# tingiskhan/pyfilter

Measured on AMD Instinct MI355X. Metric: particle-steps/sec (batch x particles x T), 1M-particle APF, higher is better.
Workload: dtype f32; 1 GPU; apf_lgo_1m: APF + lgo proposal, systematic resampling, N=1048576 particles x B=1 filters per GPU, T=250, state dim 1; parallelism=single GPU

## Files before the change

### pyfilter_amd/csrc/pf_fused.hpp

```cpp
#pragma once

namespace pf {

#define PF_STEP_B blockIdx.x
#define PF_STEP_K blockIdx.y

#ifdef PF_DEVTOOLS
#define PF_CUT(a, n) ((a).debug_cut == (n))
#define PF_STAMP(a, slot)                                                                       \
    do {                                                                                        \
        if ((a).debug_cut < 0 && !(a).finalize_only && PF_STEP_K == (unsigned)(-(a).debug_cut - 1) &&  \
            PF_STEP_B == 0 && threadIdx.x == 0)                                                 \
            (a).dbg[slot] = (unsigned long long)clock64();                                      \
    } while (0)
#else
#define PF_CUT(a, n) false
#ifdef PF_ISA_MARKS
#define PF_STAMP(a, slot) asm volatile("; PF_MARK " #slot)
#else
#define PF_STAMP(a, slot) do { } while (0)
#endif
#endif

template <typename T> struct FusedArgs {
// ... 383 lines not shown
    for (int r = 0; r < g.rounds_per_tile; ++r) {
        const int64_t r0 = base + (int64_t)r * g.round_elems;
        if (r0 >= g.N) break;
        ++rk;
        const int64_t i0 = r0 + threadIdx.x * VEC;
        const bool on = i0 < g.N;
        T rw[VEC];
#pragma unroll
        for (int j = 0; j < VEC; ++j) rw[j] = -Lim<T>::inf();
        if (on) {
            T lw[VEC], xv[D][VEC];
            if (VEC == 1) lw[0] = lw_col[i0]; else load_vec<T, VEC>(lw_col + i0, lw);
#pragma unroll
            for (int d = 0; d < D; ++d) {
                const T* xc = x_base + ((int64_t)d * g.B + b) * g.N + i0;
                if (VEC == 1) xv[d][0] = xc[0]; else load_vec<T, VEC>(xc, xv[d]);
            }
            T pre[VEC];
#pragma unroll
            for (int j = 0; j < VEC; ++j) {
                T xj[D];
#pragma unroll
                for (int d = 0; d < D; ++d) xj[d] = xv[d][j];
                UserMS<T, D> um = UserMS<T, D>::none();
                if (user && pre_on) {
                    um.gather(a.user_loc, a.user_scale, (int64_t)b * g.N, (int64_t)g.B * g.N, i0 + j, a.user_scale_percol != 0, b, g.B);
                    um.euler(xj, a.user_dt);
                }
                pre[j] = pre_on ? pre_weight<T, D>(a.md, a.proposal, cp, cc, xj, false, um) : T(0);
                if (pre_on && is_nan_or_posinf(pre[j])) acc.poison = true;
                rw[j] = pre_on ? sanitize_logw(pre[j] + lw[j]) : lw[j];
            }
            T e_unused[VEC];
            acc.template push_round<VEC>(lw, xv, false, pre, piv, e_unused);
            if (a.resampler == PF_RESAMPLE_MULTINOMIAL) {
                T ev[VEC];
                draw_exponentials<T, VEC>(a.seed + (a.seed_dev ? *a.seed_dev : 0ull), PF_STREAM_MULTINOMIAL, (uint32_t)a.step,
                                          (uint64_t)((int64_t)b * g.N + i0), ev);
#pragma unroll
                for (int j = 0; j < VEC; ++j) acc.es += (double)ev[j];
            }
        }
        chunk_scan_round<T, VEC>(rw, on, l_col + r0, threadIdx.x * VEC, r * PF_NWAVES + (threadIdx.x >> 6), use_lds ? crec : nullptr, ct_tile);
    }
    T M1, M2, F1, F2;
    acc.template finish<true>(a.part_w(a.step), b, k, g.B, g.tiles, false, red, redm, &a.poison[(a.step & 3) * g.B + b], M1, M2, F1, F2, [](T, T) {}, []() {});
    double Mc, Sc;
    finalize_chunk_table<T>(ct_tile, use_lds ? crec : nullptr, rk * PF_NWAVES, reds, redm, Mc, Sc);
    if (threadIdx.x == 0) {
        const int64_t stride = (int64_t)g.B * g.tiles, o = (int64_t)b * g.tiles + k;
        if (pre_on) {
            a.part_w(a.step)[PQ_M2 * stride + o] = Mc;
            a.part_w(a.step)[PQ_S2 * stride + o] = Sc;
        } else {
            a.part_w(a.step)[PQ_S1 * stride + o] = Sc;
        }
    }
    if (g.rounds_per_tile == 1) {
        __syncthreads();
        const int64_t i0 = base + threadIdx.x * VEC;
        if (i0 < g.N) {
            const double* cg = ct_tile + 2 * (threadIdx.x >> 6);
            const double C = cg[0], gq = cg[1];
            T v[VEC];
            if (VEC == 1) v[0] = l_col[i0]; else load_vec<T, VEC>(l_col + i0, v);
#pragma unroll
            for (int j = 0; j < VEC; ++j) v[j] = (T)(C + gq * (double)v[j]);
            if (VEC == 1) l_col[i0] = v[0]; else store_vec<T, VEC>(l_col + i0, v);
        }
    }
}

#define PF_COMBINE_ITERS (PF_MAX_TILES / PF_BLOCK)
template <typename T> __device__ __forceinline__ double pf_rcp_tot(double tot) {
    if constexpr (sizeof(T) == 4) {
        double r = __builtin_amdgcn_rcp(tot);
        r = __builtin_fma(__builtin_fma(-tot, r, 1.0), r, r);
        r = __builtin_fma(__builtin_fma(-tot, r, 1.0), r, r);
        return r;
    }
    return 1.0 / tot;
}
#define PF_PROBE_STEP 8
struct ColSums {
    double M, S, Q;
};
template <bool WITH_Q, int NX> struct ColPartials {
    double m[PF_COMBINE_ITERS], s[PF_COMBINE_ITERS], q[PF_COMBINE_ITERS];
    double x[NX ? NX : 1][PF_COMBINE_ITERS];
};
template <bool WITH_Q, int NX = 0>
__device__ __forceinline__ void load_col_partials(const double* part, int64_t stride, int64_t cb, int tiles, int slot_m,
                                                  int slot_s, int slot_x, ColPartials<WITH_Q, NX>& r) {
    const int IT = (tiles + PF_BLOCK - 1) / PF_BLOCK;
    if constexpr (PF_COMBINE_ITERS == 4 && NX == 0) {
        if (IT == 4 && (tiles & 3) == 0) {
            const int t0 = threadIdx.x * 4;
            if (t0 < tiles) {
                double a2[2], b2[2];
                const double* pm = part + slot_m * stride + cb + t0;
                load_vec<double, 2>(pm, a2); load_vec<double, 2>(pm + 2, b2);
                r.m[0] = a2[0]; r.m[1] = a2[1]; r.m[2] = b2[0]; r.m[3] = b2[1];
                const double* ps = part + slot_s * stride + cb + t0;
                load_vec<double, 2>(ps, a2); load_vec<double, 2>(ps + 2, b2);
                r.s[0] = a2[0]; r.s[1] = a2[1]; r.s[2] = b2[0]; r.s[3] = b2[1];
                if constexpr (WITH_Q) {
                    const double* pq = part + PQ_Q1 * stride + cb + t0;
                    load_vec<double, 2>(pq, a2); load_vec<double, 2>(pq + 2, b2);
                    r.q[0] = a2[0]; r.q[1] = a2[1]; r.q[2] = b2[0]; r.q[3] = b2[1];
                } else {
                    r.q[0] = r.q[1] = r.q[2] = r.q[3] = 0.0;
                }
            } else {
#pragma unroll
                for (int q = 0; q < 4; ++q) { r.m[q] = -__builtin_huge_val(); r.s[q] = 0.0; r.q[q] = 0.0; }
            }
            return;
        }
    }
#pragma unroll
    for (int q = 0; q < PF_COMBINE_ITERS; ++q) {
        const int t = threadIdx.x * IT + q;
        const bool on = q < IT && t < tiles;
        r.m[q] = on ? part[slot_m * stride + cb + t] : -__builtin_huge_val();
        r.s[q] = on ? part[slot_s * stride + cb + t] : 0.0;
        r.q[q] = (WITH_Q && on) ? part[PQ_Q1 * stride + cb + t] : 0.0;
#pragma unroll
        for (int i = 0; i < NX; ++i) r.x[i][q] = on ? part[(slot_x + i) * stride + cb + t] : 0.0;
    }
}
template <typename T, bool WITH_Q, bool TABLE, int NX = 0>
__device__ __forceinline__ ColSums column_sums(const ColPartials<WITH_Q, NX>& in, int tiles, double* ptl, double* ftl,
                                               double* redm, double* reds, double* X = nullptr) {
#pragma clang fp contract(off)
    const int lane = threadIdx.x & 63, wid = threadIdx.x >> 6;
    const int IT = (tiles + PF_BLOCK - 1) / PF_BLOCK;
    const double (&mloc)[PF_COMBINE_ITERS] = in.m;
    const double (&sloc)[PF_COMBINE_ITERS] = in.s;
    const double (&qloc)[PF_COMBINE_ITERS] = in.q;
    const double (&xloc)[NX ? NX : 1][PF_COMBINE_ITERS] = in.x;
    T mymax_t = -Lim<T>::inf();
#pragma unroll
    for (int q = 0; q < PF_COMBINE_ITERS; ++q) mymax_t = (T)mloc[q] > mymax_t ? (T)mloc[q] : mymax_t;
    const double MR = (double)block_max<T>(mymax_t, reinterpret_cast<T*>(redm));
    double incl[PF_COMBINE_ITERS], ef[PF_COMBINE_ITERS], run = 0.0, qs = 0.0;
    double xs[NX ? NX : 1];
#pragma unroll
    for (int i = 0; i < NX; ++i) xs[i] = 0.0;
#pragma unroll
    for (int q = 0; q < PF_COMBINE_ITERS; ++q) {
        ef[q] = exp_diff_t<T>(mloc[q], MR);
        run += sloc[q] * ef[q];
        incl[q] = run;
        if (WITH_Q) qs += qloc[q] * ef[q] * ef[q];
#pragma unroll
        for (int i = 0; i < NX; ++i) xs[i] += xloc[i][q] * ef[q];
    }
    const double incl_w = wave_scan_incl(run, lane);
    const double qw = WITH_Q ? wave_sum(qs) : 0.0;
#pragma unroll
    for (int i = 0; i < NX; ++i) xs[i] = wave_sum(xs[i]);
    __syncthreads();
    if (lane == 63) reds[wid] = incl_w;
    if (WITH_Q && lane == 0) reds[PF_NWAVES + wid] = qw;
    if (NX && lane == 0) {
#pragma unroll
// ... 123 lines not shown
    }
    double mv[2 * D];
    ColPartials<true, 2 * D> p1;
    ColPartials<false, 0> p2;
    load_col_partials<true, 2 * D>(a.part_r(), stride, cb, g.tiles, PQ_M1, PQ_S1, PQ_MX, p1);
    if (two) load_col_partials<false, 0>(a.part_r(), stride, cb, g.tiles, PQ_M2, PQ_S2, 0, p2);
    const ColSums c1 = column_sums<T, true, false, 2 * D>(p1, g.tiles, nullptr, nullptr, redm, red, mv);
    ColSums c2{0.0, 1.0, 0.0};
    if (two) c2 = column_sums<T, false, false>(p2, g.tiles, nullptr, nullptr, redm, red);
    const double lse_w = c1.M + log(c1.S);
    const double ess = c1.S * c1.S / c1.Q;
    bool resample = apf ? obs : (ess < a.thr_abs);
    if (a.finalize_only) resample = false;
    if (threadIdx.x == 0) {
#pragma unroll
        for (int d = 0; d < D; ++d) {
            const double dm = mv[d] / c1.S;
            double var = mv[D + d] / c1.S - dm * dm;
            if (var < 0.0) var = 0.0;
            a.means[((int64_t)step * g.B + b) * D + d] = (T)(piv[d] + dm);
            a.vars[((int64_t)step * g.B + b) * D + d] = (T)var;
        }
        if (step > 0 && !st.ll_done) {
            double ll = 0.0;
            if (st.prev_observed) {
                ll = lse_w - st.base_lse;
                if (poisoned) ll = __builtin_nan("");
            }
            a.poison[pslot * g.B + b] = 0;
            a.ll_steps[(int64_t)(step - 1) * g.B + b] = (T)ll;
            a.ll_total[b] = (T)(ll_tot + ll);
        }
        st.lse_w = lse_w;
        if (!a.finalize_only) st.resample = resample ? 1 : 0;
        st.ll_done = a.finalize_only ? 1 : 0;
        if (!a.finalize_only) {
            st.prev_observed = obs ? 1 : 0;
            st.base_lse = apf ? a.logN - ((c2.M + log(c2.S)) - lse_w) : (resample ? a.logN : lse_w);
        }
        a.stat[b] = st;
    }
}

template <typename T, int D>
__global__ __launch_bounds__(PF_BLOCK) void k_fused_book(FusedArgs<T> a) {
    __shared__ double red[(2 + 2 * D) * PF_NWAVES];
    __shared__ double redm[PF_NWAVES];
    column_bookkeeping<T, D>(a, blockIdx.y, red, redm);
}

#define PF_WAVES_D1_GENERIC 4
#define PF_WAVES_D1_MN 3
#define PF_WAVES_DN_A 3
template <typename T, int D, int MODE, int PROP, bool FAST, int SPEC, bool MULTI> struct StepWaves {
    static constexpr int value = sizeof(T) != 4 ? 1
                                 : (D == 1 && MODE == 1 && MULTI) ? PF_WAVES_D1_MN
                                 : D == 1     ? (FAST ? 4 : PF_WAVES_D1_GENERIC)
                                 : PROP == PF_PROP_LGO ? 2
                                 : (MODE == 1 || SPEC == 2) ? PF_WAVES_DN_A
                                 : 3;
};
template <typename T, int D, int VEC> struct StepShared {
    static constexpr int WIN = SearchWin<T, VEC>::WIN;
    static constexpr bool XWIN = (sizeof(T) * D <= 8);
    T* win;
    T* xwin;
    int* sh_j0;
    int* sh_cl;
    int* sh_wm;
    double* red;
    double* reds;
    T* redm;
    double* ptl;
    double* ftl;
    int* sh_plan;
    double* crec;
};
template <typename T> struct StepPlan {
    int j0, kt0;
    T ub;
    double offE, invE;
    bool resample;
    bool have_z0;
};
template <typename T, int D, int VEC, int MODE, int SPEC, bool EARLY_Z, bool MULTI>
__device__ __forceinline__ StepPlan<T> step_prologue(const FusedArgs<T>& a, const StepShared<T, D, VEC>& sh, T (&z0)[VEC][D]) {
    const Geom& g = a.g;
    const int b = PF_STEP_B, k = a.tile_of_row(PF_STEP_K);
    const int step = a.step;
    const bool obs = SPEC ? true : a.is_obs();
    const bool apf = SPEC ? (SPEC == 1) : (a.filter == PF_FILTER_APF);
    const bool two = apf && obs;
    StepPlan<T> pl{0, 0, T(0), 0.0, 0.0, false, false};
    PF_STAMP(a, 0);
#ifdef PF_DEVTOOLS
    if (a.debug_cut < 0 && threadIdx.x == 0 && b == 0 && (k % 128) == 0 && k / 128 < 8) a.dbg[16 + k / 128] = wall_clock64();
#endif
    if (apf && !obs) return pl;
    constexpr bool multinomial = MODE == 1;
    const uint64_t seed = a.seed + (a.seed_dev ? *a.seed_dev : 0ull);
    const T u_taped = (!multinomial && a.u_tape) ? a.u_tape[(int64_t)step * g.B + b] : T(0);
    const int64_t stride = (int64_t)g.B * g.tiles;
    const int64_t cb = (int64_t)b * g.tiles;
    double* const redm_d = sh.red + 2 * PF_NWAVES;
    T e0[1] = {T(0)};
    if constexpr (multinomial) {
        T tail[1];
        draw_exponentials<T, 1>(seed, PF_STREAM_MULTINOMIAL, (uint32_t)step, (uint64_t)((int64_t)g.B * g.N + b), tail);
        spacing_table(a.part_r(), stride, cb, g.tiles, (double)tail[0], sh.ptl, sh.reds);
        pl.offE = sh.ptl[k];
        pl.invE = 1.0 / sh.ptl[g.tiles + 1];
        draw_exponentials<T, 1>(seed, PF_STREAM_MULTINOMIAL, (uint32_t)step, (uint64_t)((int64_t)b * g.N + (int64_t)k * g.tile_elems), e0);
    }
    ColPartials<true, 0> p1;
    ColPartials<false, 0> p2;
    constexpr bool SHORT = MULTI;
    const bool one_tile = SHORT && g.tiles == 1 && a.debug_cut != 77;
    double m1 = 0.0, s1 = 0.0, q1 = 0.0;
    if (one_tile) {
        const double* part = a.part_r();
        m1 = part[(two ? PQ_M2 : PQ_M1) * stride + cb];
        s1 = part[(two ? PQ_S2 : PQ_S1) * stride + cb];
        q1 = two ? 0.0 : part[PQ_Q1 * stride + cb];
    }
    const bool few_tiles = SHORT && !one_tile && g.tiles <= PF_WAVE && a.debug_cut != 79;
    if (!one_tile && !few_tiles) {
        if (two) load_col_partials<false, 0>(a.part_r(), stride, cb, g.tiles, PQ_M2, PQ_S2, 0, p2);
        else load_col_partials<true, 0>(a.part_r(), stride, cb, g.tiles, PQ_M1, PQ_S1, 0, p1);
    }
    if (EARLY_Z && (SPEC || !a.z_tape)) {
        const int64_t i0 = (int64_t)k * g.tile_elems + threadIdx.x * VEC;
        if (i0 < g.N) draw_normals<T, D, VEC>(seed, PF_STREAM_NORMAL, (uint32_t)step, (uint64_t)((int64_t)b * g.N + i0), z0);
        pl.have_z0 = true;
    }
    if (one_tile) {
        if (two) {
            column_sums_one_tile<T, false>(m1, s1, q1, sh.ptl, sh.ftl);
            pl.resample = true;
        } else {
            const ColSums c = column_sums_one_tile<T, true>(m1, s1, q1, sh.ptl, sh.ftl);
            pl.resample = c.S * c.S / c.Q < a.thr_abs;
        }
    } else if (few_tiles) {
        if (two) {
            column_sums_wave<T, false>(a.part_r(), stride, cb, g.tiles, PQ_M2, PQ_S2, sh.ptl, sh.ftl);
            pl.resample = true;
        } else {
            const ColSums c = column_sums_wave<T, true>(a.part_r(), stride, cb, g.tiles, PQ_M1, PQ_S1, sh.ptl, sh.ftl);
            pl.resample = c.S * c.S / c.Q < a.thr_abs;
        }
    } else if (two) {
        column_sums<T, false, true>(p2, g.tiles, sh.ptl, sh.ftl, redm_d, sh.red);
        pl.resample = true;
    } else {
        const ColSums c = column_sums<T, true, true>(p1, g.tiles, sh.ptl, sh.ftl, redm_d, sh.red);
        pl.resample = c.S * c.S / c.Q < a.thr_abs;
    }
    PF_STAMP(a, 1);
    if (!pl.resample) return pl;
    const double* ptl = sh.ptl;
    T p;
    if constexpr (multinomial) {
        p = (T)((pl.offE + (double)e0[0]) * pl.invE);
    } else {
        pl.ub = a.u_tape ? u_taped : uniform_draw<T>(seed, PF_STREAM_UNIFORM, (uint32_t)step, (uint64_t)b);
        p = grid_position<T>((int64_t)k * g.tile_elems, pl.ub, T(g.N));
    }
    if (one_tile && a.debug_cut != 78) {
        pl.j0 = 0;
        pl.kt0 = 0;
        return pl;
    }
    if (threadIdx.x < PF_WAVE) {
        const int lane = threadIdx.x;
        int lo = 0, hi = g.tiles - 1;
        while (lo < hi) {
            const int len = hi - lo + 1;
            const int st = (len + PF_WAVE - 1) / PF_WAVE;
            int probe = lo + (lane + 1) * st - 1;
            if (probe > hi) probe = hi;
            const bool ge = (probe >= g.tiles - 1) || !((T)ptl[probe + 1] < p);
            const unsigned long long bal = __ballot(ge);
            const int f = bal ? __ffsll((long long)bal) - 1 : PF_WAVE - 1;
            int nhi = lo + (f + 1) * st - 1;
            if (nhi > hi) nhi = hi;
            lo = lo + f * st;
            if (lo > nhi) lo = nhi;
            hi = nhi;
        }
        const int kt = lo;
        const double Pk = ptl[kt], Pn = ptl[kt + 1], fk = sh.ftl[kt];
        const int64_t first = (int64_t)kt * g.tile_elems;
        const int64_t last = (first + g.tile_elems < g.N ? first + g.tile_elems : g.N) - 1;
        const T* l_col = ((step & 1) ? a.pos : a.cdf) + (int64_t)b * g.N;
        const int64_t len = last + 1 - first;
        auto cdf_at = [&](int64_t q) -> T {
            if constexpr (MULTI) {
                const double* cg = a.ctab_r(b) + 2 * (q / (PF_WAVE * VEC));
                return cdf_from_local<T>(l_col[q], cg[0], cg[1], Pk, fk, Pn, q == last, q == g.N - 1);
            } else {
                return cdf_from_local<T>(l_col[q], Pk, fk, Pn, q == last, q == g.N - 1);
            }
        };
        int64_t res;
        bool found;
        {
            float fr = (float)((double)p - Pk) * __builtin_amdgcn_rcpf((float)(Pn - Pk));
            fr = __builtin_fminf(__builtin_fmaxf(fr, 0.0f), 1.0f);
            int64_t g0 = first + (int64_t)(fr * (float)len) - (PF_WAVE / 2) * PF_PROBE_STEP;
            const int64_t g0max = last - (PF_WAVE - 1) * PF_PROBE_STEP;
            if (g0 > g0max) g0 = g0max;
            if (g0 < first) g0 = first;
            int64_t q = g0 + (int64_t)lane * PF_PROBE_STEP;
            if (q > last) q = last;
            const unsigned long long bal = __ballot(cdf_at(q) >= p);
            const int f = bal ? __ffsll((long long)bal) - 1 : 0;
            found = bal != 0 && (f > 0 || g0 == first);
            res = f > 0 ? g0 + (int64_t)(f - 1) * PF_PROBE_STEP + 1 : first;
        }
        if (!found) {
            const int64_t st = (len + PF_WAVE - 1) / PF_WAVE;
            int64_t probe = first + (lane + 1) * st - 1;
            if (probe > last) probe = last;
            const unsigned long long bal = __ballot(cdf_at(probe) >= p);
            const int f = bal ? __ffsll((long long)bal) - 1 : PF_WAVE - 1;
            res = first + (int64_t)f * st;
            if (res > last) res = last;
        }
        if (lane == 0) {
            sh.sh_plan[0] = (int)res;
            sh.sh_plan[1] = kt;
        }
    }
    __syncthreads();
    pl.j0 = sh.sh_plan[0];
    pl.kt0 = sh.sh_plan[1];
    PF_STAMP(a, 2);
    return pl;
}
template <typename T, int D, int VEC, int MODE, int PROP, bool FAST, int SPEC, int MK, bool RS, bool MULTI>
__device__ __forceinline__ void step_body(const FusedArgs<T>& a, const StepShared<T, D, VEC>& sh, const StepPlan<T>& pl,
                                          const T (&z0)[VEC][D]) {
    const int proposal = (PROP >= 0) ? PROP : a.proposal;
    ModelDesc md = a.md;
    if constexpr (!FAST && MK == 1) { md.hid_kind = PF_HID_VERHULST_EM; md.obs_kind = PF_OBS_SV; md.obs_dim = 1; }
    if constexpr (!FAST && MK == 4) { md.hid_kind = PF_HID_LORENZ63_EM; md.obs_kind = PF_OBS_LINEAR; }
    constexpr bool USER = !FAST && MK == 3;
    constexpr int WIN = StepShared<T, D, VEC>::WIN;
    constexpr int V1 = (MODE == 0) ? 1 : VEC;
    constexpr int STAGED = PF_BLOCK * (VEC + V1);
    constexpr bool XWIN = StepShared<T, D, VEC>::XWIN;
    T* const win = sh.win;
    T* const xwin = sh.xwin;
    int& sh_j0 = *sh.sh_j0;
// ... 23 lines not shown
    const double offE = pl.offE, invE = pl.invE;
    double carryE = 0.0;
    const uint64_t seed = a.seed + (a.seed_dev ? *a.seed_dev : 0ull);
    const T* z_step = (!SPEC && a.z_tape) ? a.z_tape + (int64_t)step * D * g.B * g.N : nullptr;

    ColParams<T, D> cp;
    ColConsts<T, D> cc;
    FastCol<T> fc;
    if constexpr (!FAST && D > 1) {
        load_col_params<T, D>(a, b, step, obs, cp);
        if (pre_next) cp.load_next(a.y + ((int64_t)(step + 1) * a.y_rows + (a.y_rows == 1 ? 0 : b)) * a.md.obs_dim);
    }
    const T ub = pl.ub;

    const T* x_in = a.x[slot];
    const T* lw_in = a.logw[slot] + (int64_t)b * g.N;
#ifdef PF_DEVTOOLS
    T* lw_out = a.logw[slot ^ 1] + (int64_t)b * g.N;
    int32_t* anc_col = a.anc + (int64_t)b * g.N;
#endif
    const T* cdf_col = ((step & 1) ? a.pos : a.cdf) + (int64_t)b * g.N;
    const int64_t base = (int64_t)k * g.tile_elems;
    const T nT = T(N);
    const T rcN = a.rcN;
    const bool pow2 = (N & (N - 1)) == 0;

    bool poison = false;
    PartialAcc<T, D, SPEC != 1> acc;
    acc.init();
    PF_STAMP(a, 9);
    const double* ptab_col = sh.ptl;
    const double* ftab_col = sh.ftl;
    CdfView<T> view;
    view.L = cdf_col;
    view.ptab = ptab_col;
    view.ftab = ftab_col;
    const double* const ct_col = MULTI ? a.ctab_r(b) : nullptr;
    view.ct = ct_col;
    view.chunk_elems = PF_WAVE * VEC;
    view.N = N;
    view.tile_elems = g.tile_elems;
    view.tiles = g.tiles;

    T e_rw[VEC];
    T rwn[VEC];
#pragma unroll
    for (int j = 0; j < VEC; ++j) {
        e_rw[j] = T(0);
        rwn[j] = -Lim<T>::inf();
    }
    const bool scan_next = !apf || pre_next;
    constexpr bool single = !MULTI;
    const bool use_lds = g.rounds_per_tile * PF_NWAVES <= PF_LDS_CHUNKS;
    double* const ct_tile = a.ctab_w(step + 1, b) + 2 * (int64_t)k * g.rounds_per_tile * PF_NWAVES;
    T* const l_next = ((step & 1) ? a.cdf : a.pos) + (int64_t)b * g.N;
    int rk = 0;
    for (int r = 0; r < g.rounds_per_tile; ++r) {
        const int64_t r0 = base + (int64_t)r * g.round_elems;
        if (r0 >= g.N) break;
        const int64_t i0 = r0 + tid * VEC;
        const bool on = i0 < g.N;
        if (MODE == 0 && windowed) {
            int zero[VEC];
#pragma unroll
            for (int j = 0; j < VEC; ++j) zero[j] = 0;
            if (VEC == 1) hd[tid] = 0; else store_vec<int, VEC>(hd + tid * VEC, zero);
        }
        T pv[VEC];
        if (multinomial && windowed) {
            T ev[VEC];
            double incl[VEC], local = 0.0, total;
            if (on) draw_exponentials<T, VEC>(seed, PF_STREAM_MULTINOMIAL, (uint32_t)step, (uint64_t)((int64_t)b * g.N + i0), ev);
#pragma unroll
            for (int j = 0; j < VEC; ++j) {
                local += on ? (double)ev[j] : 0.0;
                incl[j] = local;
            }
            const double excl = block_scan_excl(local, reds, total);
#pragma unroll
            for (int j = 0; j < VEC; ++j) pv[j] = (T)((offE + carryE + excl + incl[j]) * invE);
            carryE += total;
        }

        const int ws = j0 - (j0 % VEC);
        T c0[VEC], c1[V1], xa[D][VEC], xb[D][V1];
        const int ja = ws + tid * VEC, jb = ws + PF_BLOCK * VEC + tid * V1;
        const bool ina = windowed && ja < N, inb = windowed && jb < N;
        if (ina) {
            if (VEC == 1) c0[0] = cdf_col[ja]; else load_vec<T, VEC>(cdf_col + ja, c0);
            if (XWIN) {
#pragma unroll
                for (int d = 0; d < D; ++d) {
                    const T* xc = x_in + ((int64_t)d * g.B + b) * g.N + ja;
                    if (VEC == 1) xa[d][0] = xc[0]; else load_vec<T, VEC>(xc, xa[d]);
                }
            }
        }
        if (inb) {
            if (V1 == 1) c1[0] = cdf_col[jb]; else load_vec<T, V1>(cdf_col + jb, c1);
            if (XWIN) {
#pragma unroll
                for (int d = 0; d < D; ++d) {
                    const T* xc = x_in + ((int64_t)d * g.B + b) * g.N + jb;
                    if (V1 == 1) xb[d][0] = xc[0]; else load_vec<T, V1>(xc, xb[d]);
                }
            }
        }
        T lw_old[VEC];
        if (on && !resample) {
            if (VEC == 1) lw_old[0] = lw_in[i0]; else load_vec<T, VEC>(lw_in + i0, lw_old);
        }

        T zt[VEC][D];
        if (on) {
            if (z_step) {
#pragma unroll
                for (int d = 0; d < D; ++d) {
                    T zr[VEC];
                    const T* zc = z_step + ((int64_t)d * g.B + b) * g.N + i0;
                    if (VEC == 1) zr[0] = zc[0]; else load_vec<T, VEC>(zc, zr);
#pragma unroll
                    for (int j = 0; j < VEC; ++j) zt[j][d] = zr[j];
                }
            } else if (r == 0 && pl.have_z0) {
#pragma unroll
                for (int j = 0; j < VEC; ++j)
#pragma unroll
                    for (int d = 0; d < D; ++d) zt[j][d] = z0[j][d];
            } else {
                draw_normals<T, D, VEC>(seed, PF_STREAM_NORMAL, (uint32_t)step, (uint64_t)((int64_t)b * g.N + i0), zt);
            }
        }
        PF_STAMP(a, 10);
#ifdef PF_DEVTOOLS
        if (PF_CUT(a, 4)) {
            if (on) lw_out[i0] = zt[0][0] + zt[VEC - 1][D - 1];
            continue;
        }
#endif

        int idx[VEC];
        if (windowed) {
            auto map_window = [&](int w0, int wja, int wjb, bool wina, bool winb, T (&m0)[VEC], T (&m1)[V1]) {
                const int te = g.tile_elems;
                while ((unsigned)((kt0 + 1) * te) <= (unsigned)w0) ++kt0;
                int kta = kt0, ktb = kt0;
                {
                    const unsigned e1 = (unsigned)(kt0 + 1) * te, e2 = e1 + te, e3 = e2 + te;
                    kta += ((unsigned)wja >= e1) + ((unsigned)wja >= e2) + ((unsigned)wja >= e3);
                    ktb += ((unsigned)wjb >= e1) + ((unsigned)wjb >= e2) + ((unsigned)wjb >= e3);
                    if (!wina) kta = kt0;
                    if (!winb) ktb = kt0;
                }
                const double tPa = ptab_col[kta], tNa = ptab_col[kta + 1], tFa = ftab_col[kta];
                const double tPb = ptab_col[ktb], tNb = ptab_col[ktb + 1], tFb = ftab_col[ktb];
                const unsigned ea = (unsigned)(kta + 1) * te, eb = (unsigned)(ktb + 1) * te;
                const int la = (int)(ea < (unsigned)N ? ea : (unsigned)N) - 1;
                const int lb = (int)(eb < (unsigned)N ? eb : (unsigned)N) - 1;
                if constexpr (MULTI) {
                    const double* cga = ct_col + 2 * ((wina ? wja : 0) / (PF_WAVE * VEC));
                    const double* cgb = ct_col + 2 * ((winb ? wjb : 0) / (PF_WAVE * VEC));
                    const double Ca = cga[0], ga = cga[1], Cb = cgb[0], gb = cgb[1];
#pragma unroll
                    for (int j = 0; j < VEC; ++j) {
                        const bool tl = (j == VEC - 1) && (wja + j == la);
                        m0[j] = wina ? cdf_from_local<T>(m0[j], Ca, ga, tPa, tFa, tNa, tl, tl && (wja + j == N - 1)) : Lim<T>::inf();
                    }
#pragma unroll
                    for (int j = 0; j < V1; ++j)
                        m1[j] = winb ? cdf_from_local<T>(m1[j], Cb, gb, tPb, tFb, tNb, wjb + j == lb, wjb + j == N - 1) : Lim<T>::inf();
                } else {
#pragma unroll
                    for (int j = 0; j < VEC; ++j) {
                        const bool tl = (j == VEC - 1) && (wja + j == la);
                        m0[j] = wina ? cdf_from_local<T>(m0[j], tPa, tFa, tNa, tl, tl && (wja + j == N - 1)) : Lim<T>::inf();
                    }
#pragma unroll
                    for (int j = 0; j < V1; ++j)
                        m1[j] = winb ? cdf_from_local<T>(m1[j], tPb, tFb, tNb, wjb + j == lb, wjb + j == N - 1) : Lim<T>::inf();
                }
            };
            map_window(ws, ja, jb, ina, inb, c0, c1);
            if (XWIN) {
#pragma unroll
                for (int d = 0; d < D; ++d) {
                    if (ina) { if (VEC == 1) xwin[d * WIN + tid] = xa[d][0]; else store_vec<T, VEC>(xwin + d * WIN + tid * VEC, xa[d]); }
                    if (inb) { if (V1 == 1) xwin[d * WIN + PF_BLOCK * VEC + tid] = xb[d][0]; else store_vec<T, V1>(xwin + d * WIN + PF_BLOCK * VEC + tid * V1, xb[d]); }
                }
            }
            if constexpr (MODE != 0) {
                if (VEC == 1) { win[tid] = c0[0]; win[PF_BLOCK + tid] = c1[0]; }
                else { store_vec<T, VEC>(win + tid * VEC, c0); store_vec<T, VEC>(win + (PF_BLOCK + tid) * VEC, c1); }
                __syncthreads();
                T pp[VEC];
                int qq[VEC];
#pragma unroll
                for (int j = 0; j < VEC; ++j) pp[j] = multinomial ? pv[j] : grid_position<T>(i0 + j, ub, nT);
                window_lower_bound_flat<T, WIN, VEC>(win, pp, qq);
#pragma unroll
                for (int j = 0; j < VEC; ++j) {
                    const int64_t i = i0 + j;
                    int res = N - 1;
                    if (i < N) {
                        res = (qq[j] < WIN) ? ws + qq[j] : view.lower_bound(ws + WIN < N ? ws + WIN : N, pp[j], kt0);
                        if (res > N - 1) res = N - 1;
                    }
                    idx[j] = res;
                }
            } else {
                inverse_grid_round<T, VEC, V1>(c0, c1, ws, (int)r0, g.round_elems, N, ub, nT, rcN, pow2, i0, hd, sh_cl, sh_wm,
                                           [&](int it, T (&d0)[VEC], T (&d1)[V1]) -> bool {
                                               const int w0 = ws + it * STAGED;
                                               if (w0 >= N) return false;
                                               const int wja = w0 + tid * VEC, wjb = w0 + PF_BLOCK * VEC + tid * V1;
                                               const bool wina = wja < N, winb = wjb < N;
                                               if (wina) { if (VEC == 1) d0[0] = cdf_col[wja]; else load_vec<T, VEC>(cdf_col + wja, d0); }
                                               if (winb) { if (V1 == 1) d1[0] = cdf_col[wjb]; else load_vec<T, V1>(cdf_col + wjb, d1); }
                                               map_window(w0, wja, wjb, wina, winb, d0, d1);
                                               return true;
                                           },
                                           [&](int64_t i, int from) { return view.lower_bound(from, grid_position<T>(i, ub, nT), from ? kt0 : 0); },
                                           idx);
            }
            if (r + 1 < g.rounds_per_tile) {
                if (tid == PF_BLOCK - 1) sh_j0 = idx[VEC - 1];
                __syncthreads();
                j0 = sh_j0;
            }
        } else {
#pragma unroll
            for (int j = 0; j < VEC; ++j) idx[j] = (int)((i0 + j < g.N) ? (i0 + j) : (g.N - 1));
        }
        PF_STAMP(a, 11);
#ifdef PF_DEVTOOLS
        if (on && PF_CUT(a, 2)) {
            if (VEC == 1) anc_col[i0] = idx[0]; else store_vec<int, VEC>(anc_col + i0, idx);
        }
#endif

        int late;
        asm volatile("v_readfirstlane_b32 %0, %1\n\ts_and_b32 %0, %0, 0" : "=s"(late) : "v"(idx[0]) : "scc");
        using KArgs = const __attribute__((address_space(4))) FusedArgs<T>;
        KArgs* la = (KArgs*)((const_ptr<char>)__builtin_amdgcn_kernarg_segment_ptr() + late);
        T* const x_out = la->x[slot ^ 1];
        if constexpr (FAST) {
            const_ptr<T> yq = (const_ptr<T>)(uintptr_t)a.y + late;
            const int yc = a.y_rows == 1 ? 0 : b;
            const T y_t = obs ? yq[(int64_t)step * a.y_rows + yc] : T(0);
            const T y_n = pre_next ? yq[(int64_t)(step + 1) * a.y_rows + yc] : T(0);
            fc.load((const_ptr<T>)(uintptr_t)(a.cpack + (int64_t)b * PK_N) + late, y_t, y_n);
        } else if constexpr (D == 1) {
            load_col_params<T, D>(a, b, step, obs, cp, late);
            if (pre_next) cp.load_next(a.y + ((int64_t)(step + 1) * a.y_rows + (a.y_rows == 1 ? 0 : b)) * a.md.obs_dim + late);
            cc.prepare(md, cp);
            if constexpr (USER) {
                if (la->user_scale_percol) cc.prepare_user(md, cp, la->user_scale[b]);
            } else {
                __builtin_assume(cc.fast == FAST);
            }
        } else if (r == 0) {
            cc.prepare(md, cp);
            __builtin_assume(cc.fast == FAST);
        }
        T xo[D][VEC];
        if (on && !PF_CUT(a, 2)) {
            T lwo[VEC], pre_n[VEC];
            T xr[VEC][D];
            if (!resample) {
#pragma unroll
                for (int d = 0; d < D; ++d) {
                    T xv[VEC];
                    const T* xc = x_in + ((int64_t)d * g.B + b) * g.N + i0;
                    if (VEC == 1) xv[0] = xc[0]; else load_vec<T, VEC>(xc, xv);
#pragma unroll
                    for (int j = 0; j < VEC; ++j) xr[j][d] = xv[j];
                }
            } else {
#pragma unroll
                for (int j = 0; j < VEC; ++j) {
                    const int q = idx[j] - ws;
                    const bool in_lds = XWIN && windowed && q >= 0 && q < STAGED;
#pragma unroll
                    for (int d = 0; d < D; ++d)
                        xr[j][d] = in_lds ? xwin[d * WIN + q] : x_in[((int64_t)d * g.B + b) * g.N + idx[j]];
                }
            }
#pragma unroll
            for (int j = 0; j < VEC; ++j) {
                T xn[D];
                T w_new;
                UserMS<T, D> um = UserMS<T, D>::none();
                if constexpr (USER) {
                    um.gather(la->user_loc, la->user_scale, (int64_t)b * g.N, (int64_t)g.B * g.N, idx[j], la->user_scale_percol != 0, b, g.B);
                    um.euler(xr[j], la->user_dt);
                }
                if (obs) {
                    T wi, pre_anc = T(0);
                    if constexpr (FAST) {
                        if (apf) wi = fc.template sample_and_weight_apf<FAST ? MK : 0>(proposal, xr[j][0], zt[j][0], xn[0], pre_anc);
                        else wi = fc.template sample_and_weight<FAST ? MK : 0>(proposal, xr[j][0], zt[j][0], xn[0]);
                    } else {
                        wi = sample_and_weight<T, D>(md, proposal, cp, cc, xr[j], zt[j], xn, um);
                    }
                    if (apf) {
                        if constexpr (FAST) w_new = wi - pre_anc;
// ... 252 lines not shown
```

### pyfilter_amd/csrc/pf_kernels.hip

```cpp
#include <hip/hip_runtime.h>
#include <stdint.h>

#include <atomic>
#include <cstdlib>
#include <cstring>
#include <mutex>
#include <vector>

#include <type_traits>

#include "../../include/pf_amd.h"
#include "pf_device.hpp"
#include "pf_models.hpp"
#include "pf_philox.hpp"
#include "pf_linear.hpp"

namespace pf {

#define PF_MAX_TILES 1024
#define PF_TARGET_WGS 1024
#define PF_AUTO_FLAGS 128

struct Geom {
    int64_t N;
// ... 101 lines not shown
    w.off_piv0 = o;
    o = align256(o + sizeof(double) * (size_t)g.B * PF_MAXD);
    w.off_ctab = o;
    w.ctab_elems = (size_t)g.B * g.tiles * g.rounds_per_tile * PF_NWAVES * 2;
    o = align256(o + 2 * sizeof(double) * w.ctab_elems);
    w.off_clu = o;
    w.clu_bytes = (g.N > PF_CLUSTER_MIN_N && g.N <= PF_CLUSTER_MAX_N && g.N % 4 == 0 && ((g.N + 1023) / 1024) * (int64_t)g.B <= 8192)
                      ? 256 + (size_t)2 * g.B * PF_CLUSTER_NG * 64 * 16 : 0;
    o = align256(o + w.clu_bytes);
    w.off_tree = o;
    o = align256(o + sizeof(double) * (size_t)g.B * cdf_tree_total(g.N));
    w.total = o;
    return w;
}

static inline size_t ws_bound(int64_t N, int64_t B) {
    Geom g = make_geom(N, B, (int64_t)1 << 40);
    const int64_t rounds_total = (N + g.round_elems - 1) / g.round_elems;
    const size_t most_tiles = make_ws(g).total;
    g.tiles = 1;
    g.rounds_per_tile = (int)(2 * rounds_total + 2);
    const size_t most_chunks = make_ws(g).total;
    return most_tiles + most_chunks;
}

enum { PQ_M1 = 0, PQ_S1 = 1, PQ_Q1 = 2, PQ_M2 = 3, PQ_S2 = 4, PQ_E = 5, PQ_MX = 6 };

template <typename T> __device__ __forceinline__ int wave_lower_bound(const T* __restrict__ c, int n, T p, int lane) {
    int lo = 0, hi = n;
    while (hi - lo > PF_WAVE) {
        const int len = hi - lo;
        const int step = (len + PF_WAVE - 1) / PF_WAVE;
        int probe = lo + (lane + 1) * step - 1;
        if (probe > hi - 1) probe = hi - 1;
        const bool ge = c[probe] >= p;
        const unsigned long long bal = __ballot(ge);
        if (bal == 0ull) return n - 1;
        const int f = __ffsll((long long)bal) - 1;
        int nhi = lo + (f + 1) * step;
        if (nhi > hi) nhi = hi;
        lo = lo + f * step;
        hi = nhi;
    }
    const int idx = lo + lane;
    const bool ge = (idx < hi) ? (c[idx] >= p) : true;
    const unsigned long long bal = __ballot(ge);
    const int f = __ffsll((long long)bal) - 1;
    int r = lo + f;
    return r > n - 1 ? n - 1 : r;
}

template <typename T> __device__ __forceinline__ int thread_lower_bound(const T* __restrict__ c, int lo, int hi, T p) {
    while (lo < hi) {
        const int mid = (lo + hi) >> 1;
        if (c[mid] < p) lo = mid + 1; else hi = mid;
    }
    return lo;
}

template <typename T> __device__ __forceinline__ T grid_position(int64_t i, T u, T n_as_t) { return (T(i) + u) / n_as_t; }

template <typename T, bool POW2> __device__ __forceinline__ T grid_value(T x_plus_u, T nT, T rcN) {
    return POW2 ? x_plus_u * rcN : x_plus_u / nT;
}
template <typename T, bool POW2> __device__ __forceinline__ int grid_count(T c, T u, T nT, T rcN, int N) {
    T t = __builtin_fma(c, nT, -u);
    t = __builtin_fmin(__builtin_fmax(t, T(-1)), nT);
    const T fl = __builtin_floor(t);
    const T pa = grid_value<T, POW2>(fl + u, nT, rcN), pb = grid_value<T, POW2>((fl + T(1)) + u, nT, rcN);
    const int K = (int)fl + ((pa <= c) ? 1 : 0) + ((pb <= c) ? 1 : 0);
    return K < 0 ? 0 : (K > N ? N : K);
}
template <typename T, int VEC, bool POW2>
__device__ __forceinline__ void grid_counts_local(const T (&c)[VEC], T u, T nT, T rcN, int N, int r0, int RE,
                                                  int (&out)[VEC]) {
#pragma unroll
    for (int j = 0; j < VEC; ++j) {
        const int k = grid_count<T, POW2>(c[j], u, nT, rcN, N) - r0;
        out[j] = k < 0 ? 0 : (k > RE ? RE : k);
    }
}

#define PF_MAX_WINDOWS 12
template <typename T, int VEC, int V1, typename NextWindow, typename Fallback>
__device__ __forceinline__ void inverse_grid_round(const T (&c0)[VEC], const T (&c1)[V1], int ws, int r0i, int RE, int N,
                                                   T ub, T nT, T rcN, bool pow2, int64_t i0, int* hd, int* sh_cl, int* sh_wm,
                                                   NextWindow&& next_window, Fallback&& fallback, int (&idx)[VEC]) {
    constexpr int S = PF_BLOCK * (VEC + V1);
    const int tid = threadIdx.x;
    const int lane = tid & 63, wid = tid >> 6;
    const int dump = RE + lane;
    auto scatter_window = [&](const T (&w0)[VEC], const T (&w1)[V1], int qbase, int covered_before) -> int {
        int cn0[VEC], cn1[V1];
        if (pow2) {
            grid_counts_local<T, VEC, true>(w0, ub, nT, rcN, N, r0i, RE, cn0);
            grid_counts_local<T, V1, true>(w1, ub, nT, rcN, N, r0i, RE, cn1);
        } else {
            grid_counts_local<T, VEC, false>(w0, ub, nT, rcN, N, r0i, RE, cn0);
            grid_counts_local<T, V1, false>(w1, ub, nT, rcN, N, r0i, RE, cn1);
        }
        if (lane == 63) {
            sh_cl[wid] = cn0[VEC - 1];
            sh_cl[PF_NWAVES + wid] = cn1[V1 - 1];
        }
        __syncthreads();
        int pv0 = wave_prev(cn0[VEC - 1], 0), pv1 = wave_prev(cn1[V1 - 1], 0);
        if (lane == 0) {
            pv0 = wid ? sh_cl[wid - 1] : covered_before;
            pv1 = sh_cl[PF_NWAVES + wid - 1];
        }
        const int covered = sh_cl[2 * PF_NWAVES - 1];
#pragma unroll
        for (int j = 0; j < VEC; ++j) {
            const int lo0 = j ? cn0[j - 1] : pv0;
            hd[(cn0[j] > lo0) ? lo0 : dump] = qbase + tid * VEC + j + 1;
        }
#pragma unroll
        for (int j = 0; j < V1; ++j) {
            const int lo1 = j ? cn1[j - 1] : pv1;
            hd[(cn1[j] > lo1) ? lo1 : dump] = qbase + PF_BLOCK * VEC + tid * V1 + j + 1;
        }
        return covered;
    };
    int covered = scatter_window(c0, c1, 0, 0);
    int windows = 1;
    for (; windows < PF_MAX_WINDOWS && covered < RE; ++windows) {
        __syncthreads();
        T d0[VEC], d1[V1];
        if (!next_window(windows, d0, d1)) break;
        covered = scatter_window(d0, d1, windows * S, covered);
    }
    __syncthreads();
    int h[VEC];
    if (VEC == 1) h[0] = hd[tid]; else load_vec<int, VEC>(hd + tid * VEC, h);
#pragma unroll
    for (int j = 1; j < VEC; ++j) h[j] = imax(h[j], h[j - 1]);
    const int inc = wave_scan_max(h[VEC - 1]);
    if (lane == 63) sh_wm[wid] = inc;
    __syncthreads();
    int carry = wave_prev(inc, 0);
#pragma unroll
    for (int w = 0; w < PF_NWAVES - 1; ++w) carry = (w < wid) ? imax(carry, sh_wm[w]) : carry;
    const int64_t beyond = (int64_t)ws + (int64_t)windows * S;
#pragma unroll
    for (int j = 0; j < VEC; ++j) {
        const int64_t i = i0 + j;
        const int q = imax(carry, h[j]);
        int res = ws + q - 1;
        if (i < N && (tid * VEC + j >= covered || q == 0)) res = fallback(i, (q == 0) ? 0 : (int)(beyond < N ? beyond : N));
        idx[j] = (i < N && res < N) ? res : N - 1;
    }
}

template <typename T, int VEC> struct SearchWin {
    static constexpr int WIN = 2 * PF_BLOCK * VEC;
};

template <typename T, int WIN, int VEC>
__device__ __forceinline__ void window_lower_bound_flat(const T* win, const T (&p)[VEC], int (&out)[VEC]) {
    static_assert((WIN & (WIN - 1)) == 0, "window size must be a power of two");
    const unsigned char* const wb = reinterpret_cast<const unsigned char*>(win);
#pragma unroll
    for (int j = 0; j < VEC; ++j) out[j] = 0;
#pragma unroll
    for (int step = WIN / 2; step >= 1; step >>= 1) {
        T v[VEC];
#pragma unroll
        for (int j = 0; j < VEC; ++j) v[j] = *reinterpret_cast<const T*>(wb + out[j] + (step - 1) * (int)sizeof(T));
#pragma unroll
        for (int j = 0; j < VEC; ++j) out[j] += (v[j] < p[j]) ? step * (int)sizeof(T) : 0;
    }
#pragma unroll
    for (int j = 0; j < VEC; ++j) {
        out[j] += (*reinterpret_cast<const T*>(wb + out[j]) < p[j]) ? (int)sizeof(T) : 0;
        out[j] /= (int)sizeof(T);
    }
}

template <typename T, int VEC>
__device__ __forceinline__ void systematic_round(const T* __restrict__ cdf_col, int N, int64_t i0, T u,
                                                 const T* __restrict__ u_elem, T* win, int* sh_j0, int (&idx)[VEC]) {
    constexpr int WIN = SearchWin<T, VEC>::WIN;
    const int tid = threadIdx.x;
    const int j0 = *sh_j0;
    const int ws = j0 - (j0 % VEC);
    {
        T v0[VEC], v1[VEC];
        const int ja = ws + tid * VEC, jb = ws + (PF_BLOCK + tid) * VEC;
        const bool ina = ja < N, inb = jb < N;
        if (ina) { if (VEC == 1) v0[0] = cdf_col[ja]; else load_vec<T, VEC>(cdf_col + ja, v0); }
        if (inb) { if (VEC == 1) v1[0] = cdf_col[jb]; else load_vec<T, VEC>(cdf_col + jb, v1); }
#pragma unroll
        for (int j = 0; j < VEC; ++j) {
            if (!ina) v0[j] = Lim<T>::inf();
            if (!inb) v1[j] = Lim<T>::inf();
        }
        if (VEC == 1) { win[tid] = v0[0]; win[PF_BLOCK + tid] = v1[0]; }
        else { store_vec<T, VEC>(win + tid * VEC, v0); store_vec<T, VEC>(win + (PF_BLOCK + tid) * VEC, v1); }
    }
    __syncthreads();
    const T nT = T(N);
    T pp[VEC];
    int qq[VEC];
#pragma unroll
    for (int j = 0; j < VEC; ++j) pp[j] = (i0 + j < N) ? grid_position<T>(i0 + j, u_elem ? u_elem[i0 + j] : u, nT) : T(0);
    window_lower_bound_flat<T, WIN, VEC>(win, pp, qq);
#pragma unroll
    for (int j = 0; j < VEC; ++j) {
        const int64_t i = i0 + j;
        int res = N - 1;
        if (i < N) {
            res = (qq[j] < WIN) ? ws + qq[j] : thread_lower_bound<T>(cdf_col, ws + WIN < N ? ws + WIN : N, N, pp[j]);
            if (res > N - 1) res = N - 1;
        }
        idx[j] = res;
    }
    __syncthreads();
    if (tid == PF_BLOCK - 1) *sh_j0 = idx[VEC - 1];
    __syncthreads();
}


template <typename T, int VEC>
__device__ __forceinline__ void reduce_logw_body(T* __restrict__ logw, int sanitize, const uint8_t* colmask,
                                                 double* __restrict__ part, const Geom& g, int b, int k) {
    __shared__ double red[4 * PF_NWAVES];
    __shared__ T redm[PF_NWAVES];
    if (colmask && !colmask[b]) return;
    T* col = logw + (int64_t)b * g.N;
    OnlineLse<T> acc;
    acc.init();
    double q = 0.0;
    const int64_t base = (int64_t)k * g.tile_elems;
    for (int r = 0; r < g.rounds_per_tile; ++r) {
// ... 2482 lines not shown
```

Before: 78.75 billion particle-steps/s.

## Speculatively estimate resampling window start by interpolation within tile CDF table

For the systematic, single-filter, VEC=4 path, the prologue now estimates the resampling window start by linearly interpolating the target position inside the located tile, minus a safety margin. This replaces the wave-wide probe of the tile's CDF entries. The first window's counts are checked, and if the guess overshoots, the block falls back to the original probe search and reloads the window. This removes global-memory probe loads and a ballot round from the common path. In exchange it adds a verdict check with a barrier and a costly fallback path for steps where the estimate misses.

```diff
diff --git a/pyfilter_amd/csrc/pf_fused.hpp b/pyfilter_amd/csrc/pf_fused.hpp
--- a/pyfilter_amd/csrc/pf_fused.hpp
+++ b/pyfilter_amd/csrc/pf_fused.hpp
@@ -489,6 +489,18 @@
     return 1.0 / tot;
 }
 #define PF_PROBE_STEP 8
+#ifndef PF_WINDOW_MARGIN
+#define PF_WINDOW_MARGIN 96
+#endif
+template <int VEC, int MODE, bool MULTI> struct WindowStart {
+    static constexpr bool speculative = !MULTI && VEC == 4 && MODE == 0;
+};
+static_assert(PF_WINDOW_MARGIN % 4 == 0 && PF_WINDOW_MARGIN < PF_BLOCK, "the margin comes out of the window's 256 spare entries");
+#ifndef PF_WINDOW_START_BROADCAST
+#define PF_WINDOW_START_BROADCAST 0
+#endif
+#define PF_CUT_FORCE_PROBE 76
+#define PF_CUT_COUNT_STARTS 75
 struct ColSums {
     double M, S, Q;
 };
@@ -778,7 +790,59 @@
     double offE, invE;
     bool resample;
     bool have_z0;
+    bool spec;
 };
+template <typename T> __device__ __forceinline__ int table_tile_search(const double* ptl, int tiles, T p, int lane) {
+    int lo = 0, hi = tiles - 1;
+    while (lo < hi) {
+        const int len = hi - lo + 1;
+        const int st = (len + PF_WAVE - 1) / PF_WAVE;
+        int probe = lo + (lane + 1) * st - 1;
+        if (probe > hi) probe = hi;
+        const bool ge = (probe >= tiles - 1) || !((T)ptl[probe + 1] < p);
+        const unsigned long long bal = __ballot(ge);
+        const int f = bal ? __ffsll((long long)bal) - 1 : PF_WAVE - 1;
+        int nhi = lo + (f + 1) * st - 1;
+        if (nhi > hi) nhi = hi;
+        lo = lo + f * st;
+        if (lo > nhi) lo = nhi;
+        hi = nhi;
+    }
+    return lo;
+}
+__device__ __forceinline__ float table_tile_fraction(double p, double Pk, double Pn) {
+    const float fr = (float)(p - Pk) * __builtin_amdgcn_rcpf((float)(Pn - Pk));
+    return __builtin_fminf(__builtin_fmaxf(fr, 0.0f), 1.0f);
+}
+template <typename T>
+__device__ __forceinline__ int probe_window_start(const FusedArgs<T>& a, const double* ptl, const double* ftl, int b, int step,
+                                                  T p, int kt, int lane) {
+    const Geom& g = a.g;
+    const double Pk = ptl[kt], Pn = ptl[kt + 1], fk = ftl[kt];
+    const int N = (int)g.N;
+    const int first = kt * g.tile_elems;
+    const int last = (first + g.tile_elems < N ? first + g.tile_elems : N) - 1;
+    const int len = last + 1 - first;
+    const T* l_col = ((step & 1) ? a.pos : a.cdf) + (int64_t)b * g.N;
+    auto cdf_at = [&](int q) -> T { return cdf_from_local<T>(l_col[q], Pk, fk, Pn, q == last, q == N - 1); };
+    int g0 = first + (int)(table_tile_fraction((double)p, Pk, Pn) * (float)len) - (PF_WAVE / 2) * PF_PROBE_STEP;
+    const int g0max = last - (PF_WAVE - 1) * PF_PROBE_STEP;
+    if (g0 > g0max) g0 = g0max;
+    if (g0 < first) g0 = first;
+    int q = g0 + lane * PF_PROBE_STEP;
+    if (q > last) q = last;
+    unsigned long long bal = __ballot(cdf_at(q) >= p);
+    int f = bal ? __ffsll((long long)bal) - 1 : 0;
+    if (bal != 0 && (f > 0 || g0 == first))
+        return f > 0 ? g0 + (f - 1) * PF_PROBE_STEP + 1 : first;
+    const int st = (len + PF_WAVE - 1) / PF_WAVE;
+    int probe = first + (lane + 1) * st - 1;
+    if (probe > last) probe = last;
+    bal = __ballot(cdf_at(probe) >= p);
+    f = bal ? __ffsll((long long)bal) - 1 : PF_WAVE - 1;
+    const int res = first + f * st;
+    return res > last ? last : res;
+}
 template <typename T, int D, int VEC, int MODE, int SPEC, bool EARLY_Z, bool MULTI>
 __device__ __forceinline__ StepPlan<T> step_prologue(const FusedArgs<T>& a, const StepShared<T, D, VEC>& sh, T (&z0)[VEC][D]) {
     const Geom& g = a.g;
@@ -787,7 +851,7 @@
     const bool obs = SPEC ? true : a.is_obs();
     const bool apf = SPEC ? (SPEC == 1) : (a.filter == PF_FILTER_APF);
     const bool two = apf && obs;
-    StepPlan<T> pl{0, 0, T(0), 0.0, 0.0, false, false};
+    StepPlan<T> pl{0, 0, T(0), 0.0, 0.0, false, false, false};
     PF_STAMP(a, 0);
 #ifdef PF_DEVTOOLS
     if (a.debug_cut < 0 && threadIdx.x == 0 && b == 0 && (k % 128) == 0 && k / 128 < 8) a.dbg[16 + k / 128] = wall_clock64();
@@ -866,6 +930,32 @@
         pl.j0 = 0;
         pl.kt0 = 0;
         return pl;
+    }
+    if constexpr (WindowStart<VEC, MODE, MULTI>::speculative) {
+        if (!PF_CUT(a, PF_CUT_FORCE_PROBE)) {
+            auto table_start = [&](int lane, int& kt) -> int {
+                kt = table_tile_search<T>(ptl, g.tiles, p, lane);
+                const int first = kt * g.tile_elems;
+                const int len = first + g.tile_elems < (int)g.N ? g.tile_elems : (int)g.N - first;
+                const int est = first + (int)(table_tile_fraction((double)p, ptl[kt], ptl[kt + 1]) * (float)len);
+                return est - PF_WINDOW_MARGIN < first ? first : (est - PF_WINDOW_MARGIN) & ~(VEC - 1);
+            };
+#if PF_WINDOW_START_BROADCAST
+            if (threadIdx.x < PF_WAVE) {
+                int kt;
+                const int ws = table_start((int)threadIdx.x, kt);
+                if (threadIdx.x == 0) { sh.sh_plan[0] = ws; sh.sh_plan[1] = kt; }
+            }
+            __syncthreads();
+            pl.j0 = sh.sh_plan[0];
+            pl.kt0 = sh.sh_plan[1];
+#else
+            pl.j0 = table_start((int)(threadIdx.x & (PF_WAVE - 1)), pl.kt0);
+#endif
+            pl.spec = pl.j0 != pl.kt0 * g.tile_elems;
+            PF_STAMP(a, 2);
+            return pl;
+        }
     }
     if (threadIdx.x < PF_WAVE) {
         const int lane = threadIdx.x;
@@ -1055,7 +1145,7 @@
             carryE += total;
         }
 
-        const int ws = j0 - (j0 % VEC);
+        int ws = j0 - (j0 % VEC);
         T c0[VEC], c1[V1], xa[D][VEC], xb[D][V1];
         const int ja = ws + tid * VEC, jb = ws + PF_BLOCK * VEC + tid * V1;
         const bool ina = windowed && ja < N, inb = windowed && jb < N;
@@ -1181,19 +1271,68 @@
                     idx[j] = res;
                 }
             } else {
-                inverse_grid_round<T, VEC, V1>(c0, c1, ws, (int)r0, g.round_elems, N, ub, nT, rcN, pow2, i0, hd, sh_cl, sh_wm,
-                                           [&](int it, T (&d0)[VEC], T (&d1)[V1]) -> bool {
-                                               const int w0 = ws + it * STAGED;
-                                               if (w0 >= N) return false;
-                                               const int wja = w0 + tid * VEC, wjb = w0 + PF_BLOCK * VEC + tid * V1;
-                                               const bool wina = wja < N, winb = wjb < N;
-                                               if (wina) { if (VEC == 1) d0[0] = cdf_col[wja]; else load_vec<T, VEC>(cdf_col + wja, d0); }
-                                               if (winb) { if (V1 == 1) d1[0] = cdf_col[wjb]; else load_vec<T, V1>(cdf_col + wjb, d1); }
-                                               map_window(w0, wja, wjb, wina, winb, d0, d1);
-                                               return true;
-                                           },
-                                           [&](int64_t i, int from) { return view.lower_bound(from, grid_position<T>(i, ub, nT), from ? kt0 : 0); },
-                                           idx);
+                auto next_window = [&](int it, T (&d0)[VEC], T (&d1)[V1]) -> bool {
+                    const int w0 = ws + it * STAGED;
+                    if (w0 >= N) return false;
+                    const int wja = w0 + tid * VEC, wjb = w0 + PF_BLOCK * VEC + tid * V1;
+                    const bool wina = wja < N, winb = wjb < N;
+                    if (wina) { if (VEC == 1) d0[0] = cdf_col[wja]; else load_vec<T, VEC>(cdf_col + wja, d0); }
+                    if (winb) { if (V1 == 1) d1[0] = cdf_col[wjb]; else load_vec<T, V1>(cdf_col + wjb, d1); }
+                    map_window(w0, wja, wjb, wina, winb, d0, d1);
+                    return true;
+                };
+                auto search = [&](int64_t i, int from) { return view.lower_bound(from, grid_position<T>(i, ub, nT), from ? kt0 : 0); };
+                if constexpr (WindowStart<VEC, MODE, MULTI>::speculative) {
+                    int windows = inverse_grid_round<T, VEC, V1, true>(c0, c1, ws, (int)r0, g.round_elems, N, ub, nT, rcN, pow2, i0, hd, sh_cl,
+                                                                       sh_wm, next_window, search, idx, pl.spec, &sh_j0);
+                    const bool accepted = windows != 0;
+                    if (!accepted) {
+                        if (tid < PF_WAVE) {
+                            const int res = probe_window_start<T>(a, ptab_col, ftab_col, b, step, grid_position<T>(base, ub, nT), kt0, tid);
+                            if (tid == 0) sh.sh_plan[0] = res;
+                        }
+                        __syncthreads();
+                        j0 = sh.sh_plan[0];
+                        ws = j0 - (j0 % VEC);
+                        const int fja = ws + tid * VEC, fjb = ws + PF_BLOCK * VEC + tid * V1;
+                        const bool fina = fja < N, finb = fjb < N;
+                        if (fina) {
+                            load_vec<T, VEC>(cdf_col + fja, c0);
+                            if (XWIN) {
+#pragma unroll
+                                for (int d = 0; d < D; ++d) load_vec<T, VEC>(x_in + ((int64_t)d * g.B + b) * g.N + fja, xa[d]);
+                            }
+                        }
+                        if (finb) {
+                            c1[0] = cdf_col[fjb];
+                            if (XWIN) {
+#pragma unroll
+                                for (int d = 0; d < D; ++d) xb[d][0] = x_in[((int64_t)d * g.B + b) * g.N + fjb];
+                            }
+                        }
+                        map_window(ws, fja, fjb, fina, finb, c0, c1);
+                        if (XWIN) {
+#pragma unroll
+                            for (int d = 0; d < D; ++d) {
+                                if (fina) store_vec<T, VEC>(xwin + d * WIN + tid * VEC, xa[d]);
+                                if (finb) xwin[d * WIN + PF_BLOCK * VEC + tid] = xb[d][0];
+                            }
+                        }
+                        windows = inverse_grid_round<T, VEC, V1>(c0, c1, ws, (int)r0, g.round_elems, N, ub, nT, rcN, pow2, i0, hd, sh_cl, sh_wm,
+                                                                 next_window, search, idx);
+                    }
+#ifdef PF_DEVTOOLS
+                    if (tid == 0 && (PF_CUT(a, PF_CUT_COUNT_STARTS) || PF_CUT(a, PF_CUT_FORCE_PROBE))) {
+                        atomicAdd(&a.dbg[accepted ? 3 : 4], 1ull);
+                        if (windows > 1) atomicAdd(&a.dbg[5], 1ull);
+                        if (accepted && pl.spec) atomicAdd(&a.dbg[6], 1ull);
+                        if (accepted && windows == 1) atomicAdd(&a.dbg[7], 1ull);
+                    }
+#endif
+                } else {
+                    inverse_grid_round<T, VEC, V1>(c0, c1, ws, (int)r0, g.round_elems, N, ub, nT, rcN, pow2, i0, hd, sh_cl, sh_wm, next_window,
+                                                   search, idx);
+                }
             }
             if (r + 1 < g.rounds_per_tile) {
                 if (tid == PF_BLOCK - 1) sh_j0 = idx[VEC - 1];
diff --git a/pyfilter_amd/csrc/pf_kernels.hip b/pyfilter_amd/csrc/pf_kernels.hip
--- a/pyfilter_amd/csrc/pf_kernels.hip
+++ b/pyfilter_amd/csrc/pf_kernels.hip
@@ -207,15 +207,16 @@
 }
 
 #define PF_MAX_WINDOWS 12
-template <typename T, int VEC, int V1, typename NextWindow, typename Fallback>
-__device__ __forceinline__ void inverse_grid_round(const T (&c0)[VEC], const T (&c1)[V1], int ws, int r0i, int RE, int N,
-                                                   T ub, T nT, T rcN, bool pow2, int64_t i0, int* hd, int* sh_cl, int* sh_wm,
-                                                   NextWindow&& next_window, Fallback&& fallback, int (&idx)[VEC]) {
+template <typename T, int VEC, int V1, bool CHECK = false, typename NextWindow, typename Fallback>
+__device__ __forceinline__ int inverse_grid_round(const T (&c0)[VEC], const T (&c1)[V1], int ws, int r0i, int RE, int N,
+                                                  T ub, T nT, T rcN, bool pow2, int64_t i0, int* hd, int* sh_cl, int* sh_wm,
+                                                  NextWindow&& next_window, Fallback&& fallback, int (&idx)[VEC],
+                                                  bool check = false, int* verdict = nullptr) {
     constexpr int S = PF_BLOCK * (VEC + V1);
     const int tid = threadIdx.x;
     const int lane = tid & 63, wid = tid >> 6;
     const int dump = RE + lane;
-    auto scatter_window = [&](const T (&w0)[VEC], const T (&w1)[V1], int qbase, int covered_before) -> int {
+    auto scatter_window = [&](const T (&w0)[VEC], const T (&w1)[V1], int qbase, int covered_before, auto first_window) -> int {
         int cn0[VEC], cn1[V1];
         if (pow2) {
             grid_counts_local<T, VEC, true>(w0, ub, nT, rcN, N, r0i, RE, cn0);
@@ -228,7 +229,13 @@
             sh_cl[wid] = cn0[VEC - 1];
             sh_cl[PF_NWAVES + wid] = cn1[V1 - 1];
         }
+        if constexpr (CHECK && decltype(first_window)::value) {
+            if (check && tid == 0) *verdict = cn0[0];
+        }
         __syncthreads();
+        if constexpr (CHECK && decltype(first_window)::value) {
+            if (check && *verdict != 0) return -1;
+        }
         int pv0 = wave_prev(cn0[VEC - 1], 0), pv1 = wave_prev(cn1[V1 - 1], 0);
         if (lane == 0) {
             pv0 = wid ? sh_cl[wid - 1] : covered_before;
@@ -247,13 +254,16 @@
         }
         return covered;
     };
-    int covered = scatter_window(c0, c1, 0, 0);
+    int covered = scatter_window(c0, c1, 0, 0, std::true_type{});
+    if constexpr (CHECK) {
+        if (covered < 0) return 0;
+    }
     int windows = 1;
     for (; windows < PF_MAX_WINDOWS && covered < RE; ++windows) {
         __syncthreads();
         T d0[VEC], d1[V1];
         if (!next_window(windows, d0, d1)) break;
-        covered = scatter_window(d0, d1, windows * S, covered);
+        covered = scatter_window(d0, d1, windows * S, covered, std::false_type{});
     }
     __syncthreads();
     int h[VEC];
@@ -275,6 +285,7 @@
         if (i < N && (tid * VEC + j >= covered || q == 0)) res = fallback(i, (q == 0) ? 0 : (int)(beyond < N ? beyond : N));
         idx[j] = (i < N && res < N) ? res : N - 1;
     }
+    return windows;
 }
 
 template <typename T, int VEC> struct SearchWin {
```

New measurement: 79.37 billion particle-steps/s (median of 6 runs). No clear change (+0.8%).
